# genglongling/EE274_ConvexCaldera_LLM_quantization

Hardware: AMD Instinct MI355X
Metric: weight matrices/sec (4096x4096, rank-128, Q=2-bit) + Frob err vs ref (higher is better)
Workload: dtype f32 (fp16 W in; fp32-grade split-fp16 MFMA products, fp64 small solves; int2 codes)

## Files before the change

### ee274_convexcaldera_llm_quantization_amd/csrc/cq_sgram.hip

```cpp
#include "cq_common.h"

namespace cq {

constexpr int SG_SLICE = 64;

__device__ __forceinline__ uint32_t sg_nz_mask(uint32_t word) {
    const uint32_t x = word ^ 0x55555555u;
    return (x | (x >> 1)) & 0x55555555u;
}

__device__ __forceinline__ uint32_t sg_field(uint32_t word, int u) {
    return (word >> (8 * (u >> 2) + 6 - 2 * (u & 3))) & 3u;
}

__device__ __forceinline__ int sg_u_of_bit(int p) { return 4 * (p >> 3) + ((6 - (p & 7)) >> 1); }

__global__ __launch_bounds__(256) void sgram_count_kernel(const uint8_t* __restrict__ packed, int64_t k, int64_t L,
                                                          int32_t* __restrict__ row_nnz, const _Float16* __restrict__ W,
                                                          const float* __restrict__ qscale,
                                                          const float* __restrict__ wcol, double* __restrict__ row_corr,
                                                          int64_t Lh, int32_t* __restrict__ row_nnz1, int64_t wcs) {
    const int lane = threadIdx.x & 63;
    const int64_t j = (int64_t)blockIdx.x * 4 + (threadIdx.x >> 6);
    const int64_t b = blockIdx.y;
    if (wcol) wcol += b * wcs;
    if (j >= k) return;
    const uint32_t* row = reinterpret_cast<const uint32_t*>(packed + b * (k * L / 4) + j * (L / 4));
    const int64_t nw = L / 16;
    uint32_t cnt = 0, cnt1 = 0;
    double corr = 0.0;
    const double s = W ? (double)qscale[b] : 0.0;
    const _Float16* Wr = W ? W + b * k * L + j * L : nullptr;
    const int64_t nw1 = Lh / 16;
    for (int64_t w = lane; w < nw; w += 64) {
        const uint32_t word = row[w];
        uint32_t nz = sg_nz_mask(word);
        cnt += __popc(nz);
        if (w < nw1) cnt1 += __popc(nz);
        if (W) {
            while (nz) {
                const int p = __builtin_ctz(nz);
                nz &= nz - 1u;
                const int64_t l = 16 * w + sg_u_of_bit(p);
                const double c = (double)((int)((word >> p) & 3u) - 1);
                const double t = s * s - 2.0 * s * c * (double)(float)Wr[l];
                corr += wcol ? (double)wcol[l] * t : t;
            }
        }
    }
    cnt = wave_sum(cnt);
    if (lane == 0) row_nnz[b * k + j] = (int32_t)cnt;
    if (row_nnz1) {
// ... 243 lines not shown
            }
        }
        cntr[r] = cnt;
        __builtin_amdgcn_wave_barrier();
    }
    const int g = lane >> 4, u = lane & 15;
    const int q = (int)((p0 + g) & 15);
    for (int h = 0; h < np; ++h) {
        int myc = 0, mys = 0, mycnt = 0;
        uint32_t* myout = nullptr;
        int T = 0;
#pragma unroll
        for (int r = 0; r < SG_FILL_RW; ++r) {
            const int cn = cntr[r] <= 0 ? 0 : (h ? cntr[r] - c1r[r] : c1r[r]);
            if (g == r) {
                mycnt = cn;
                myout = outr[r] ? outr[r] + (h ? w1r[r] * SG_SLICE : 0) : nullptr;
            }
            T = cn > T ? cn : T;
        }
        if (mycnt > 0) {
            myc = rcb[wv][g][h][u];
            mys = rsb[wv][g][h][u];
        }
        int taken = 0;
        for (int t = 0; t < T; ++t) {
            const int d = (q + t) & 15;
            const int remd = __shfl(myc - taken, 16 * g + d, 64);
            int key = ((myc - taken) << 4) | (15 - u);
#pragma unroll
            for (int o = 8; o > 0; o >>= 1) key = max(key, __shfl_xor(key, o, 64));
            const int sel = remd > 0 ? d : 15 - (key & 15);
            const int at = __shfl(mys + taken, 16 * g + sel, 64);
            if (t < mycnt) {
                if (u == 0) myout[(int64_t)t * SG_SLICE] = grp[wv][g][at];
                if (u == sel) ++taken;
            }
        }
    }
#pragma unroll
    for (int r = 0; r < SG_FILL_RW; ++r) {
        if (!outr[r]) continue;
        const int tot = cntr[r] < 0 ? -cntr[r] : cntr[r];
        for (int64_t t = c1r[r] + lane; t < w1r[r]; t += 64) outr[r][t * SG_SLICE] = 1u;
        if (split) {
            const uint32_t pad = (uint32_t)(Lh << 2) | 1u;
            for (int64_t t = w1r[r] + (tot - c1r[r]) + lane; t < widr[r]; t += 64) outr[r][t * SG_SLICE] = pad;
        }
    }
}

constexpr int SG_PF = 6;
constexpr int SG_WAVES = 16, SG_THREADS = 64 * SG_WAVES;

template <int R>
__device__ __forceinline__ int64_t sg_slab_at(int64_t L, int64_t l, int r) {
    constexpr int PL = R < 4 ? R : 4;
    return (int64_t)(r / PL) * PL * L + l * PL + (r % PL);
}

template <int R>
__device__ __forceinline__ void sg_slice(const float* __restrict__ slab, int64_t L, const uint32_t* __restrict__ ep,
                                         int64_t width, float (&acc)[R], int64_t lbase = 0) {
#pragma unroll
    for (int r = 0; r < R; ++r) acc[r] = 0.f;
    constexpr int PL = R < 4 ? R : 4;
    auto fma_entry = [&](uint32_t e) {
        const float c = (float)((int)(e & 3u) - 1);
        const int64_t l = (int64_t)(e >> 2) - lbase;
#pragma unroll
        for (int pl = 0; pl < R / PL; ++pl) {
            const float* v = slab + (int64_t)pl * PL * L + l * PL;
#pragma unroll
            for (int r = 0; r < PL; ++r) acc[pl * PL + r] = __builtin_fmaf(c, v[r], acc[pl * PL + r]);
        }
    };
    int64_t t = 0;
    if (width >= SG_PF) {
        uint32_t cur[SG_PF];
#pragma unroll
        for (int q = 0; q < SG_PF; ++q) cur[q] = ep[q * SG_SLICE];
        for (t = SG_PF; t + SG_PF <= width; t += SG_PF) {
            uint32_t nxt[SG_PF];
#pragma unroll
            for (int q = 0; q < SG_PF; ++q) nxt[q] = ep[(t + q) * SG_SLICE];
#pragma unroll
            for (int q = 0; q < SG_PF; ++q) fma_entry(cur[q]);
#pragma unroll
            for (int q = 0; q < SG_PF; ++q) cur[q] = nxt[q];
        }
#pragma unroll
        for (int q = 0; q < SG_PF; ++q) fma_entry(cur[q]);
    }
    for (; t < width; ++t) fma_entry(ep[t * SG_SLICE]);
}

template <int R, int NSW, bool SPLIT = false>
__global__ __launch_bounds__(1024) void sgram_spmm_kernel(const _Float16* __restrict__ W, const uint8_t* __restrict__ packed,
                                                         const float* __restrict__ qscale, const float* __restrict__ wcol,
                                                         int64_t k, int64_t L, const uint32_t* __restrict__ ell,
                                                         const int32_t* __restrict__ perm,
                                                         const int64_t* __restrict__ slice_off,
                                                         const int32_t* __restrict__ slice_w1, int64_t Lh,
                                                         int64_t stride_ell, float* __restrict__ P, int64_t wcs) {
    extern __shared__ __attribute__((aligned(16))) float slab[];
    const int64_t b = blockIdx.y;
    if (wcol) wcol += b * wcs;
    const int64_t i0 = (int64_t)blockIdx.x * R;
    const float hs = 0.5f * qscale[b];
    const int64_t KL = k * L;
    const int64_t Ls = SPLIT ? Lh : L;
    constexpr int PL = R < 4 ? R : 4;
    auto stage = [&](int64_t la, int64_t lb) {
#pragma unroll
    for (int pl = 0; pl < R / PL; ++pl) {
        for (int64_t l0 = la + (int64_t)threadIdx.x * 8; l0 < lb; l0 += SG_THREADS * 8) {
            float e[PL][8];
#pragma unroll
            for (int r = 0; r < PL; ++r) {
                const int64_t i = i0 + pl * PL + r;
                if (i < k) {
                    const int64_t el = b * KL + i * L + l0;
                    const uint4 raw = *reinterpret_cast<const uint4*>(W + el);
                    const _Float16* hv = reinterpret_cast<const _Float16*>(&raw);
                    const uint16_t two = *reinterpret_cast<const uint16_t*>(packed + el / 4);
#pragma unroll
                    for (int u = 0; u < 8; ++u) {
                        const uint32_t byte = (u < 4) ? (two & 0xffu) : (two >> 8);
                        const float c = (float)((int)((byte >> (6 - 2 * (u & 3))) & 3u) - 1);
                        e[r][u] = (float)hv[u] - hs * c;
                        if (wcol) e[r][u] *= wcol[l0 + u];
                    }
                } else {
#pragma unroll
                    for (int u = 0; u < 8; ++u) e[r][u] = 0.f;
                }
            }
            const int rot = threadIdx.x & 7;
#pragma unroll
            for (int sh = 1; sh < 8; sh <<= 1) {
                if (rot & sh) {
#pragma unroll
                    for (int r = 0; r < PL; ++r) {
                        float t8[8];
#pragma unroll
                        for (int u = 0; u < 8; ++u) t8[u] = e[r][(u + sh) & 7];
#pragma unroll
                        for (int u = 0; u < 8; ++u) e[r][u] = t8[u];
                    }
                }
            }
#pragma unroll
            for (int u = 0; u < 8; ++u) {
                float* dst = slab + (int64_t)pl * PL * Ls + (l0 - la + ((u + rot) & 7)) * PL;
                if constexpr (PL == 4) *reinterpret_cast<float4*>(dst) = make_float4(e[0][u], e[1][u], e[2][u], e[3][u]);
                else *reinterpret_cast<float2*>(dst) = make_float2(e[0][u], e[1][u]);
            }
        }
    }
    };
    stage(0, SPLIT ? Lh : L);
    __syncthreads();
    const int lane = threadIdx.x & 63, wv = threadIdx.x >> 6;
    const int64_t ns = (k + SG_SLICE - 1) / SG_SLICE;
    const int64_t* so = slice_off + b * (ns + 1);
    const uint32_t* eb = ell + b * stride_ell + lane;
    const int32_t* pm = perm + b * k;
    float* Pb = P + b * k * k;
    if constexpr (NSW > 0) {
        float acc[NSW][R];
#pragma unroll
        for (int q = 0; q < NSW; ++q) {
            const int64_t s = wv + SG_WAVES * q;
            if (s < ns) sg_slice<R>(slab, L, eb + so[s] * SG_SLICE, so[s + 1] - so[s], acc[q]);
        }
        __syncthreads();
#pragma unroll
        for (int q = 0; q < NSW; ++q) {
            const int64_t p = (wv + SG_WAVES * q) * SG_SLICE + lane;
            if (p < k) {
                float* dst = slab + pm[p] * R;
#pragma unroll
                for (int pl = 0; pl < R / PL; ++pl) {
                    if constexpr (PL == 4)
                        *reinterpret_cast<float4*>(dst + 4 * pl) = make_float4(acc[q][4 * pl], acc[q][4 * pl + 1],
                                                                              acc[q][4 * pl + 2], acc[q][4 * pl + 3]);
                    else *reinterpret_cast<float2*>(dst) = make_float2(acc[q][0], acc[q][1]);
                }
            }
        }
        __syncthreads();
        for (int64_t j = threadIdx.x; j < k; j += SG_THREADS) {
            float v[R];
#pragma unroll
            for (int pl = 0; pl < R / PL; ++pl) {
                if constexpr (PL == 4) {
                    const float4 x = *reinterpret_cast<const float4*>(slab + j * R + 4 * pl);
                    v[4 * pl] = x.x; v[4 * pl + 1] = x.y; v[4 * pl + 2] = x.z; v[4 * pl + 3] = x.w;
                } else {
                    const float2 x = *reinterpret_cast<const float2*>(slab + j * R);
                    v[0] = x.x; v[1] = x.y;
                }
            }
#pragma unroll
            for (int r = 0; r < R; ++r)
                if (i0 + r < k) Pb[(i0 + r) * k + j] = v[r];
        }
    } else if constexpr (NSW < 0) {
        float* outb = slab + (int64_t)R * Ls;
        const int32_t* w1 = SPLIT ? slice_w1 + b * ns : nullptr;
        for (int64_t s = wv; s < ns; s += SG_WAVES) {
            float acc[R];
            sg_slice<R>(slab, Ls, eb + so[s] * SG_SLICE, SPLIT ? w1[s] : so[s + 1] - so[s], acc);
            const int64_t p = s * SG_SLICE + lane;
            if (p < k) {
#pragma unroll
                for (int r = 0; r < R; ++r) outb[(int64_t)pm[p] * R + r] = acc[r];
            }
        }
        if constexpr (SPLIT) {
            __syncthreads();
            stage(Lh, L);
            __syncthreads();
            for (int64_t s = wv; s < ns; s += SG_WAVES) {
                float acc[R];
                sg_slice<R>(slab, Ls, eb + (so[s] + w1[s]) * SG_SLICE, so[s + 1] - so[s] - w1[s], acc, Lh);
                const int64_t p = s * SG_SLICE + lane;
                if (p < k) {
#pragma unroll
                    for (int r = 0; r < R; ++r) outb[(int64_t)pm[p] * R + r] += acc[r];
                }
            }
        }
        __syncthreads();
        for (int64_t j = threadIdx.x; j < k; j += SG_THREADS) {
#pragma unroll
            for (int r = 0; r < R; ++r)
                if (i0 + r < k) Pb[(i0 + r) * k + j] = outb[j * R + r];
        }
    } else {
        for (int64_t s = wv; s < ns; s += SG_WAVES) {
            float acc[R];
            sg_slice<R>(slab, L, eb + so[s] * SG_SLICE, so[s + 1] - so[s], acc);
            const int64_t p = s * SG_SLICE + lane;
            if (p < k) {
                const int64_t j = pm[p];
#pragma unroll
                for (int r = 0; r < R; ++r)
                    if (i0 + r < k) Pb[(i0 + r) * k + j] = acc[r];
            }
        }
    }
}

__device__ __forceinline__ float sg_split_scale(double bound) {
    int e = 0;
    if (bound > 0.0 && isfinite(bound)) frexp(bound, &e);
    return ldexpf(1.f, 14 - e);
}

__global__ __launch_bounds__(256) void sgram_combine_kernel(const float* __restrict__ A, const float* __restrict__ P,
                                                            const float* __restrict__ qscale, int64_t k,
                                                            const double* __restrict__ bound, float out_scale,
                                                            _Float16* __restrict__ Gh, _Float16* __restrict__ Gl,
                                                            float* __restrict__ scale_out, float* __restrict__ inv_out,
                                                            float* __restrict__ G32) {
    __shared__ float pt[64][65];
    const int64_t b = blockIdx.y;
    const int64_t nt = k / 64;
    int64_t t = blockIdx.x, I = 0;
    while (t >= nt - I) { t -= nt - I; ++I; }
    const int64_t J = I + t;
    const int64_t I0 = I * 64, J0 = J * 64;
    const float s = qscale[b];
    const float gs = sg_split_scale(bound[b]);
    if (blockIdx.x == 0 && threadIdx.x == 0) {
        scale_out[b] = gs;
        inv_out[b] = 1.f / (gs * out_scale);
    }
    const int64_t KK = k * k;
    const float* Pb = P + b * KK;
    const int tx = threadIdx.x & 15, ty = threadIdx.x >> 4;
    for (int a = ty; a < 64; a += 16) {
        const float4 v = *reinterpret_cast<const float4*>(Pb + (J0 + a) * k + I0 + 4 * tx);
        pt[a][4 * tx] = v.x; pt[a][4 * tx + 1] = v.y; pt[a][4 * tx + 2] = v.z; pt[a][4 * tx + 3] = v.w;
    }
    __syncthreads();
    float g[4][4];
#pragma unroll
    for (int q = 0; q < 4; ++q) {
        const int a = ty + 16 * q;
        const float4 av = *reinterpret_cast<const float4*>(A + b * KK + (I0 + a) * k + J0 + 4 * tx);
        const float4 pv = *reinterpret_cast<const float4*>(Pb + (I0 + a) * k + J0 + 4 * tx);
        const float aa[4] = {av.x, av.y, av.z, av.w}, pp[4] = {pv.x, pv.y, pv.z, pv.w};
#pragma unroll
        for (int u = 0; u < 4; ++u) g[q][u] = aa[u] - s * (pp[u] + pt[4 * tx + u][a]);
// ... 348 lines not shown
    CQ_REQUIRE(bits == 2, "cq_sgram_count: 2-bit codes only");
    CQ_REQUIRE(batch > 0 && batch < 65536 && k > 0 && L > 0 && L % 64 == 0, "cq_sgram_count: bad shape");
    CQ_REQUIRE(!W || (qscale && corr_ws && corr_out), "cq_sgram_count: the norm correction needs qscale, corr_ws, corr_out");
    CQ_REQUIRE(Lh >= L || (Lh > 0 && Lh % 64 == 0 && 2 * Lh >= L && row_nnz1 && slice_w1),
               "cq_sgram_count: an l-split needs Lh % 64 == 0, Lh >= L / 2, row_nnz1 and slice_w1");
    const bool split = Lh < L;
    hipStream_t s = as_stream(stream);
    sgram_count_kernel<<<dim3((unsigned)ceil_div(k, 4), (unsigned)batch), 256, 0, s>>>(
        packed, k, L, row_nnz, reinterpret_cast<const _Float16*>(W), qscale, wcol, corr_ws, split ? Lh : L,
        split ? row_nnz1 : nullptr, wcol_stride);
    sgram_slices_kernel<<<(unsigned)batch, 256, 0, s>>>(row_nnz, k, perm, slice_off, total, W ? corr_ws : nullptr,
                                                        corr_out, split ? row_nnz1 : nullptr, slice_w1);
    return check_launch("cq_sgram_count");
}

int cq_sgram_fill(const uint8_t* packed, int bits, int64_t batch, int64_t k, int64_t L, const int32_t* row_nnz,
                  const int32_t* perm, const int64_t* slice_off, const int32_t* slice_w1, int64_t Lh,
                  int64_t stride_ell, uint32_t* ell, void* stream) {
    CQ_REQUIRE(packed && row_nnz && perm && slice_off && ell, "cq_sgram_fill: null argument");
    CQ_REQUIRE(bits == 2, "cq_sgram_fill: 2-bit codes only");
    CQ_REQUIRE(batch > 0 && batch < 65536 && k > 0 && L > 0 && L % 64 == 0 && L < (1ll << 29),
               "cq_sgram_fill: bad shape");
    CQ_REQUIRE(Lh >= L || (Lh > 0 && Lh % 64 == 0 && 2 * Lh >= L && slice_w1), "cq_sgram_fill: bad l-split");
    sgram_fill_kernel<<<dim3((unsigned)ceil_div(k, 4 * SG_FILL_RW), (unsigned)batch), 256, 0, as_stream(stream)>>>(
        packed, k, L, row_nnz, perm, slice_off, slice_w1, Lh < L ? Lh : L, stride_ell, ell);
    return check_launch("cq_sgram_fill");
}

int cq_sgram_rows(int64_t L) {
    for (int r : {8, 4, 2})
        if ((size_t)L * r * sizeof(float) <= 150 * 1024) return r;
    return 0;
}

int64_t cq_sgram_split(int64_t k, int64_t L) {
    if (cq_sgram_rows(L) != 2 || L % 64) return L;
    const int64_t Lh = ceil_div(L / 2, (int64_t)64) * 64;
    return ((size_t)Lh * 4 + (size_t)k * 4) * sizeof(float) <= 150 * 1024 ? Lh : L;
}

int cq_sgram_spmm(int dtype, const void* W, const uint8_t* packed, const float* qscale, const float* wcol,
                  int64_t wcol_stride, int64_t batch, int64_t k, int64_t L, const uint32_t* ell, const int32_t* perm,
                  const int64_t* slice_off, const int32_t* slice_w1, int64_t Lh, int64_t stride_ell, float* P,
                  void* stream) {
    CQ_REQUIRE(W && packed && qscale && ell && perm && slice_off && P, "cq_sgram_spmm: null argument");
    CQ_REQUIRE(dtype == CQ_F16, "cq_sgram_spmm: fp16 W only");
    CQ_REQUIRE(batch > 0 && batch < 65536 && k > 0 && L % 64 == 0, "cq_sgram_spmm: bad shape");
    hipStream_t s = as_stream(stream);
    const _Float16* Wh = reinterpret_cast<const _Float16*>(W);
    if (Lh < L) {
        CQ_REQUIRE(Lh == cq_sgram_split(k, L) && slice_w1, "cq_sgram_spmm: Lh must be cq_sgram_split(k, L)");
        const size_t lds = ((size_t)Lh * 4 + (size_t)k * 4) * sizeof(float);
        sgram_spmm_kernel<4, -1, true><<<dim3((unsigned)ceil_div(k, 4), (unsigned)batch), SG_THREADS, lds, s>>>(
            Wh, packed, qscale, wcol, k, L, ell, perm, slice_off, slice_w1, Lh, stride_ell, P, wcol_stride);
        return check_launch("cq_sgram_spmm");
    }
    const int R = cq_sgram_rows(L);
    CQ_REQUIRE(R > 0, "cq_sgram_spmm: rows of %lld values do not fit the LDS", (long long)L);
    size_t lds = (size_t)L * R * sizeof(float);
    const dim3 grid((unsigned)ceil_div(k, R), (unsigned)batch);
    const int64_t nsw = ceil_div(ceil_div(k, SG_SLICE), SG_WAVES);
    const bool held = k <= L && nsw * R <= 32 && R == 8;
    const bool ldsout = !held && R < 8 && lds + (size_t)k * R * sizeof(float) <= 150 * 1024;
    if (ldsout) lds += (size_t)k * R * sizeof(float);
#define CQ_SP(RR, NN) sgram_spmm_kernel<RR, NN><<<grid, SG_THREADS, lds, s>>>(Wh, packed, qscale, wcol, k, L, ell, \
                                                                             perm, slice_off, nullptr, L, stride_ell, P, \
                                                                             wcol_stride)
    if (R == 8) {
        if (held) CQ_SP(8, 4); else CQ_SP(8, 0);
    } else if (R == 4) {
        if (ldsout) CQ_SP(4, -1); else CQ_SP(4, 0);
    } else {
        if (ldsout) CQ_SP(2, -1); else CQ_SP(2, 0);
    }
#undef CQ_SP
    return check_launch("cq_sgram_spmm");
}

int cq_sgram_combine(const float* A, const float* P, const float* qscale, int64_t batch, int64_t k,
                     const double* bound, float out_scale, uint16_t* Gh, uint16_t* Gl, float* scale_out,
                     float* inv_out, float* G32, void* stream) {
    CQ_REQUIRE(A && P && qscale && bound && Gh && Gl && scale_out && inv_out, "cq_sgram_combine: null argument");
    CQ_REQUIRE(batch > 0 && batch < 65536 && k > 0 && k % 64 == 0 && out_scale > 0.f, "cq_sgram_combine: bad shape");
    const int64_t nt = k / 64;
    sgram_combine_kernel<<<dim3((unsigned)(nt * (nt + 1) / 2), (unsigned)batch), 256, 0, as_stream(stream)>>>(
        A, P, qscale, k, bound, out_scale, reinterpret_cast<_Float16*>(Gh), reinterpret_cast<_Float16*>(Gl),
        scale_out, inv_out, G32);
    return check_launch("cq_sgram_combine");
}

}
```

### ee274_convexcaldera_llm_quantization_amd/csrc/cq_small.hip

```cpp
#include "cq_common.h"

namespace cq {

constexpr int GT = 64;
constexpr int GK = 32;
constexpr int kGramThreads = 256;

__global__ __launch_bounds__(kGramThreads) void gram_f64_kernel(
    int64_t M, int64_t N, int64_t K, int64_t kchunk, int splits, const float* __restrict__ A,
    int ta, int64_t lda, int64_t sa, const float* __restrict__ B, int tb, int64_t ldb, int64_t sb,
    double* __restrict__ part) {
    __shared__ float As[GK][GT + 1];
    __shared__ float Bs[GK][GT + 1];
    const int64_t b = blockIdx.z / splits;
    const int split = blockIdx.z % splits;
    const int64_t i0 = (int64_t)blockIdx.y * GT, j0 = (int64_t)blockIdx.x * GT;
    const float* Ab = A + b * sa;
    const float* Bb = B + b * sb;
    const int tx = threadIdx.x & 15, ty = threadIdx.x >> 4;
    double acc[4][4];
#pragma unroll
    for (int u = 0; u < 4; ++u)
#pragma unroll
        for (int v = 0; v < 4; ++v) acc[u][v] = 0.0;
// ... 7 lines not shown
            if (gk < kend && gi < M) v = ta ? Ab[gi * lda + gk] : Ab[gk * lda + gi];
            As[kk][ii] = v;
            int jj;
            if (!tb) { kk = e / GT; jj = e % GT; } else { jj = e / GK; kk = e % GK; }
            const int64_t gk2 = k0 + kk, gj = j0 + jj;
            float w = 0.f;
            if (gk2 < kend && gj < N) w = tb ? Bb[gj * ldb + gk2] : Bb[gk2 * ldb + gj];
            Bs[kk][jj] = w;
        }
        __syncthreads();
#pragma unroll 4
        for (int kk = 0; kk < GK; ++kk) {
            double av[4], bv[4];
#pragma unroll
            for (int u = 0; u < 4; ++u) av[u] = (double)As[kk][ty * 4 + u];
#pragma unroll
            for (int v = 0; v < 4; ++v) bv[v] = (double)Bs[kk][tx * 4 + v];
#pragma unroll
            for (int u = 0; u < 4; ++u)
#pragma unroll
                for (int v = 0; v < 4; ++v) acc[u][v] = fma(av[u], bv[v], acc[u][v]);
        }
        __syncthreads();
    }
    double* P = part + ((int64_t)b * splits + split) * M * N;
#pragma unroll
    for (int u = 0; u < 4; ++u)
#pragma unroll
        for (int v = 0; v < 4; ++v) {
            const int64_t i = i0 + ty * 4 + u, j = j0 + tx * 4 + v;
            if (i < M && j < N) P[i * N + j] = acc[u][v];
        }
}

__global__ void gram_reduce_kernel(const double* __restrict__ part, int64_t MN, int splits,
                                   int64_t batch, double* __restrict__ C) {
    const int64_t total = batch * MN;
    for (int64_t e = (int64_t)blockIdx.x * blockDim.x + threadIdx.x; e < total;
         e += (int64_t)gridDim.x * blockDim.x) {
        const int64_t b = e / MN, o = e % MN;
        double s = 0.0;
        for (int t = 0; t < splits; ++t) s += part[(b * splits + t) * MN + o];
        C[e] = s;
    }
}


using f64x4v = __attribute__((ext_vector_type(4))) double;

template <bool TK>
__global__ __launch_bounds__(kGramThreads) void gram_f64_mfma_kernel(
    int64_t M, int64_t N, int64_t K, int64_t kchunk, int splits, const float* __restrict__ A,
    int64_t lda, int64_t sa, const float* __restrict__ B, int64_t ldb, int64_t sb, int sym,
    double* __restrict__ part) {
    constexpr int GP = TK ? GT + 4 : GT + 16;
    __shared__ float As[2][GK][GP];
    __shared__ float Bs[2][GK][GP];
    const int64_t b = blockIdx.z / splits;
    const int split = blockIdx.z % splits;
    if (sym && blockIdx.x < blockIdx.y) return;
    const int64_t i0 = (int64_t)blockIdx.y * GT, j0 = (int64_t)blockIdx.x * GT;
    const float* Ab = A + b * sa;
    const float* Bb = B + b * sb;
    const int t = threadIdx.x, lane = t & 63, wid = t >> 6;
    const int wi = wid >> 1, wj = wid & 1;
    const int lr = t >> 4, lc = (t & 15) * 4;
    const int tr = t >> 3, tk = (t & 7) * 4;
    const int64_t kbeg = split * kchunk, kend = min(K, kbeg + kchunk);
    auto ld4 = [&](const float* base, int64_t ld, int64_t lim, int64_t k, int64_t c0) -> float4 {
        float4 v = make_float4(0.f, 0.f, 0.f, 0.f);
        if (k < kend) {
            const float* src = base + k * ld + c0;
            if (c0 + 3 < lim) v = *reinterpret_cast<const float4*>(src);
            else {
                if (c0 < lim) v.x = src[0];
                if (c0 + 1 < lim) v.y = src[1];
                if (c0 + 2 < lim) v.z = src[2];
            }
        }
        return v;
    };
    f64x4v acc[2][2];
#pragma unroll
    for (int u = 0; u < 2; ++u)
#pragma unroll
        for (int v = 0; v < 2; ++v) acc[u][v] = f64x4v{0.0, 0.0, 0.0, 0.0};
    float4 ra[2], rb[2];
    auto ld4t = [&](const float* base, int64_t ld, int64_t lim, int64_t row, int64_t k) -> float4 {
        float4 v = make_float4(0.f, 0.f, 0.f, 0.f);
        if (row < lim && k < kend) {
            const float* src = base + row * ld + k;
            if (k + 3 < kend) v = *reinterpret_cast<const float4*>(src);
            else {
                v.x = src[0];
                if (k + 1 < kend) v.y = src[1];
                if (k + 2 < kend) v.z = src[2];
            }
        }
        return v;
    };
    auto fetch = [&](int64_t k0) {
#pragma unroll
        for (int h = 0; h < 2; ++h) {
            if constexpr (TK) {
                ra[h] = ld4t(Ab, lda, M, i0 + tr + 32 * h, k0 + tk);
                rb[h] = ld4t(Bb, ldb, N, j0 + tr + 32 * h, k0 + tk);
            } else {
                ra[h] = ld4(Ab, lda, M, k0 + lr + 16 * h, i0 + lc);
                rb[h] = ld4(Bb, ldb, N, k0 + lr + 16 * h, j0 + lc);
            }
        }
    };
    auto stash = [&](int buf) {
#pragma unroll
        for (int h = 0; h < 2; ++h) {
            if constexpr (TK) {
                const int c = tr + 32 * h;
                As[buf][tk + 0][c] = ra[h].x; As[buf][tk + 1][c] = ra[h].y;
                As[buf][tk + 2][c] = ra[h].z; As[buf][tk + 3][c] = ra[h].w;
                Bs[buf][tk + 0][c] = rb[h].x; Bs[buf][tk + 1][c] = rb[h].y;
                Bs[buf][tk + 2][c] = rb[h].z; Bs[buf][tk + 3][c] = rb[h].w;
            } else {
                *reinterpret_cast<float4*>(&As[buf][lr + 16 * h][lc]) = ra[h];
                *reinterpret_cast<float4*>(&Bs[buf][lr + 16 * h][lc]) = rb[h];
            }
        }
    };
    const int nsl = (int)ceil_div(kend - kbeg, GK);
    if (nsl > 0) { fetch(kbeg); stash(0); }
    __syncthreads();
    const int li = lane & 15, lk = lane >> 4;
    for (int sl = 0; sl < nsl; ++sl) {
        const int cur = sl & 1;
        if (sl + 1 < nsl) fetch(kbeg + (int64_t)(sl + 1) * GK);
#pragma unroll
        for (int kk = 0; kk < GK; kk += 4) {
            double a0 = (double)As[cur][kk + lk][32 * wi + li];
            double a1 = (double)As[cur][kk + lk][32 * wi + 16 + li];
            double b0 = (double)Bs[cur][kk + lk][32 * wj + li];
            double b1 = (double)Bs[cur][kk + lk][32 * wj + 16 + li];
            acc[0][0] = __builtin_amdgcn_mfma_f64_16x16x4f64(a0, b0, acc[0][0], 0, 0, 0);
            acc[0][1] = __builtin_amdgcn_mfma_f64_16x16x4f64(a0, b1, acc[0][1], 0, 0, 0);
            acc[1][0] = __builtin_amdgcn_mfma_f64_16x16x4f64(a1, b0, acc[1][0], 0, 0, 0);
            acc[1][1] = __builtin_amdgcn_mfma_f64_16x16x4f64(a1, b1, acc[1][1], 0, 0, 0);
        }
        if (sl + 1 < nsl) stash(1 - cur);
        __syncthreads();
    }
    double* P = part + ((int64_t)b * splits + split) * M * N;
#pragma unroll
    for (int u = 0; u < 2; ++u)
#pragma unroll
        for (int v = 0; v < 2; ++v)
#pragma unroll
            for (int r = 0; r < 4; ++r) {
                const int64_t i = i0 + 32 * wi + 16 * u + lk + 4 * r;
                const int64_t j = j0 + 32 * wj + 16 * v + li;
                if (i < M && j < N) P[i * N + j] = acc[u][v][r];
            }
}

__global__ void gram_reduce_sym_kernel(const double* __restrict__ part, int64_t M, int splits,
                                       int64_t batch, double* __restrict__ C) {
    const int64_t MN = M * M, total = batch * MN;
    for (int64_t e = (int64_t)blockIdx.x * blockDim.x + threadIdx.x; e < total;
         e += (int64_t)gridDim.x * blockDim.x) {
        const int64_t b = e / MN, o = e % MN, i = o / M, j = o % M;
        const int64_t src = (i / GT > j / GT) ? j * M + i : o;
        double s = 0.0;
        for (int t2 = 0; t2 < splits; ++t2) s += part[(b * splits + t2) * MN + src];
        C[e] = s;
    }
}

static int gram_splits(int64_t M, int64_t N, int64_t K, int64_t batch) {
    const int64_t tiles = ceil_div(M, GT) * ceil_div(N, GT) * batch;
    int64_t s = ceil_div(1024, tiles);
    s = std::min<int64_t>(s, std::max<int64_t>(1, K / 256));
    return (int)std::max<int64_t>(1, std::min<int64_t>(s, 64));
}

template <int PPT, int RPT, int JBR, int NTH>
__global__ __launch_bounds__(NTH) void jacobi_reg_kernel(const double* __restrict__ A_all,
                                                                    int p, int max_sweeps, double tol,
                                                                    double* __restrict__ evals,
                                                                    float* __restrict__ V32,
                                                                    double* __restrict__ V64,
                                                                    int* __restrict__ sweeps_out) {
    extern __shared__ __attribute__((aligned(16))) char smem_raw[];
    const int P = p + (p & 1);
    const int H = P / 2;
    double2* csn = reinterpret_cast<double2*>(smem_raw);
    int4* lohi = reinterpret_cast<int4*>(csn + H);
    int* flp = reinterpret_cast<int*>(lohi + H);
    int* seat = flp + H;
    int* seat2 = seat + P;
    int* rnk = seat2 + P;
    double* a = reinterpret_cast<double*>(rnk + P + ((9 * H + 3 * P) & 1));
    __shared__ double red[16];
    __shared__ int stop;
    const int64_t b = blockIdx.x;
    const double* Ag = A_all + b * (int64_t)p * p;
    const int tid = threadIdx.x, lane = tid & 63, wid = tid >> 6;
    const bool wantv = V32 != nullptr || V64 != nullptr;
    const int pg = lane & 31;
    const int rg = 2 * wid + (lane >> 5);
    const int k0 = pg * PPT, x0 = rg * RPT;
    auto pk = [p](int i, int j) -> int {
        if (i > j) { const int t = i; i = j; j = t; }
        return i * p - ((i * (i - 1)) >> 1) + (j - i);
    };
// ... 629 lines not shown
}

__global__ void ritz_prod_final_kernel(const double* part, int nchunks, int64_t p, int64_t r,
                                       const double* theta, const double* ysq, float* out) {
    __shared__ double red[16];
    const int64_t b = blockIdx.x;
    const double t0 = fabs(theta[b * p]), tp = theta[b * p + p - 1];
    double acc = 0.0;
    for (int64_t c = threadIdx.x; c < r; c += blockDim.x) {
        double s = 0.0;
        for (int t = 0; t < nchunks; ++t) s += part[(b * nchunks + t) * r + c];
        const double th = fmax(theta[b * p + c], 0.0);
        const double gap = fmax(th - tp, 1e-3 * t0);
        acc += s * th / (gap * gap);
    }
    acc = wave_sum(acc);
    if ((threadIdx.x & 63) == 0) red[threadIdx.x >> 6] = acc;
    __syncthreads();
    if (threadIdx.x == 0) {
        double a = 0.0;
        for (int i = 0; i < (int)(blockDim.x >> 6); ++i) a += red[i];
        const double y2 = ysq[b];
        out[b] = (float)(y2 > 0 ? sqrt(a / y2) : sqrt(a));
    }
}

}

using namespace cq;

extern "C" {

size_t cq_gram_f64_workspace(int64_t M, int64_t N, int64_t K, int64_t batch) {
    return (size_t)batch * gram_splits(M, N, K, batch) * M * N * sizeof(double);
}

int cq_gram_f64(int64_t M, int64_t N, int64_t K, int64_t batch, const float* A, int trans_a,
                int64_t lda, int64_t stride_a, const float* B, int trans_b, int64_t ldb,
                int64_t stride_b, double* C, void* ws, size_t ws_bytes, void* stream) {
    CQ_REQUIRE(A && B && C && M > 0 && N > 0 && K > 0 && batch > 0, "cq_gram_f64: bad args");
    const int splits = gram_splits(M, N, K, batch);
    if (!ws || ws_bytes < cq_gram_f64_workspace(M, N, K, batch))
        return set_error(CQ_EWORKSPACE, "cq_gram_f64: workspace too small");
    CQ_REQUIRE(batch * splits <= 65535, "cq_gram_f64: batch too large");
    const int64_t kchunk = ceil_div(ceil_div(K, splits), GK) * GK;
    hipStream_t s = as_stream(stream);
    dim3 grid((unsigned)ceil_div(N, GT), (unsigned)ceil_div(M, GT), (unsigned)(batch * splits));
    const int64_t tot = batch * M * N;
    const unsigned rgrid = (unsigned)std::min<int64_t>(ceil_div(tot, 256), 4096);
    const bool al4 = lda % 4 == 0 && ldb % 4 == 0 && stride_a % 4 == 0 && stride_b % 4 == 0 &&
                     reinterpret_cast<uintptr_t>(A) % 16 == 0 && reinterpret_cast<uintptr_t>(B) % 16 == 0;
    if (al4 && trans_a == trans_b) {
        const int sym = (A == B && lda == ldb && stride_a == stride_b && M == N) ? 1 : 0;
        if (trans_a)
            gram_f64_mfma_kernel<true><<<grid, kGramThreads, 0, s>>>(M, N, K, kchunk, splits, A, lda, stride_a, B,
                                                                     ldb, stride_b, sym, reinterpret_cast<double*>(ws));
        else
            gram_f64_mfma_kernel<false><<<grid, kGramThreads, 0, s>>>(M, N, K, kchunk, splits, A, lda, stride_a, B,
                                                                      ldb, stride_b, sym, reinterpret_cast<double*>(ws));
        if (sym)
            gram_reduce_sym_kernel<<<rgrid, 256, 0, s>>>(reinterpret_cast<double*>(ws), M, splits, batch, C);
        else
            gram_reduce_kernel<<<rgrid, 256, 0, s>>>(reinterpret_cast<double*>(ws), M * N, splits, batch, C);
        return check_launch("cq_gram_f64");
    }
    gram_f64_kernel<<<grid, kGramThreads, 0, s>>>(M, N, K, kchunk, splits, A, trans_a, lda,
                                                   stride_a, B, trans_b, ldb, stride_b,
                                                   reinterpret_cast<double*>(ws));
    gram_reduce_kernel<<<rgrid, 256, 0, s>>>(reinterpret_cast<double*>(ws), M * N, splits, batch, C);
    return check_launch("cq_gram_f64");
}

int cq_spd_whiten(double* S, int64_t p, int64_t batch, float* Wt32, double* Wt64, int* info,
                  void* stream) {
    return cq_spd_whiten_rcond(S, p, batch, 1e-30, Wt32, Wt64, info, stream);
}

int cq_spd_whiten_rcond(double* S, int64_t p, int64_t batch, double rcond2, float* Wt32, double* Wt64, int* info,
                        void* stream) {
    CQ_REQUIRE(S && p > 0 && batch > 0 && info && Wt64, "cq_spd_whiten: bad args (Wt64 is required scratch)");
    CQ_REQUIRE(rcond2 >= 0.0, "cq_spd_whiten: rcond2 must be >= 0");
    hipStream_t s = as_stream(stream);
    const size_t wsm = (size_t)(p + 2 * 32 * 33 + 32) * sizeof(double);
    const size_t wlm = wsm + (size_t)32 * wm_pitch((int)p) * sizeof(double);
    CQ_REQUIRE(wsm <= 64 * 1024, "cq_spd_whiten: p too large");
    if (wlm <= 150 * 1024)
        spd_whiten_mfma_kernel<true><<<(unsigned)batch, kWmThreads, wlm, s>>>(S, (int)p, rcond2, Wt64, Wt32, info);
    else
        spd_whiten_mfma_kernel<false><<<(unsigned)batch, kWmThreads, wsm, s>>>(S, (int)p, rcond2, Wt64, Wt32, info);
    return check_launch("cq_spd_whiten");
}

size_t cq_jacobi_workspace(int64_t p, int64_t batch) {
    if (p > kBlockJacobiMinP) return cq::bj_workspace(p, batch);
    return 16;
}

int cq_jacobi_eigh(double* A, int64_t p, int64_t batch, int max_sweeps, double tol, double* evals,
                   float* V32, double* V64, int* sweeps_out, void* ws, size_t ws_bytes,
                   void* stream) {
    CQ_REQUIRE(A && evals && p > 0 && batch > 0 && max_sweeps > 0, "cq_jacobi_eigh: bad args");
    CQ_REQUIRE(p <= 4096, "cq_jacobi_eigh: p too large");
    if (!ws || ws_bytes < cq_jacobi_workspace(p, batch))
        return set_error(CQ_EWORKSPACE, "cq_jacobi_eigh: workspace too small");
    hipStream_t s = as_stream(stream);
    if (p > kBlockJacobiMinP)
        return cq::bj_eigh(A, p, batch, max_sweeps, tol, evals, V32, V64, sweeps_out, ws, ws_bytes, s);
    const size_t lreg = jacobi_reg_bytes((int)p);
    CQ_REQUIRE(lreg <= 160 * 1024, "cq_jacobi_eigh: LDS budget");
    if (p <= 64)
        jacobi_reg_kernel<1, 2, 2, 1024><<<(unsigned)batch, 1024, lreg, s>>>(A, (int)p, max_sweeps, tol, evals, V32, V64, sweeps_out);
    else if (p <= 128)
// ... 75 lines not shown
```

Measured before the change: 350.3.

## Persist sgram SpMM blocks over multiple row tiles with prefetched staging; skip gram reduce

The held-accumulator SpMM path now has each block process up to nb consecutive row tiles. The global loads for the next tile are issued before the sparse FMA phase so they overlap with compute, and the slice metadata is loaded once per block. Staging now uses register lane rotation through alignbit instead of float shuffles. Wave-to-slice assignment is serpentine to balance load. Separately, the fp64 gram kernel writes straight into C, mirroring symmetric tiles, when there is only one split, which removes the reduce launch. The cost is higher register pressure, extra barriers, and a grid that can go below one block per tile.

```diff
diff --git a/ee274_convexcaldera_llm_quantization_amd/csrc/cq_sgram.hip b/ee274_convexcaldera_llm_quantization_amd/csrc/cq_sgram.hip
--- a/ee274_convexcaldera_llm_quantization_amd/csrc/cq_sgram.hip
+++ b/ee274_convexcaldera_llm_quantization_amd/csrc/cq_sgram.hip
@@ -1,3 +1,5 @@
+#include <algorithm>
+
 #include "cq_common.h"
 
 namespace cq {
@@ -347,6 +349,7 @@
 
 constexpr int SG_PF = 6;
 constexpr int SG_WAVES = 16, SG_THREADS = 64 * SG_WAVES;
+constexpr int64_t SG_NB_MAX = 8;
 
 template <int R>
 __device__ __forceinline__ int64_t sg_slab_at(int64_t L, int64_t l, int r) {
@@ -388,6 +391,15 @@
         for (int q = 0; q < SG_PF; ++q) fma_entry(cur[q]);
     }
     for (; t < width; ++t) fma_entry(ep[t * SG_SLICE]);
+}
+
+struct SgStageRegs {
+    uint4 raw[4];
+    uint32_t two[4];
+};
+
+__device__ __forceinline__ int64_t sg_wave_slice(int wv, int q) {
+    return (int64_t)SG_WAVES * q + ((q & 1) ? SG_WAVES - 1 - wv : wv);
 }
 
 template <int R, int NSW, bool SPLIT = false>
@@ -397,146 +409,215 @@
                                                          const int32_t* __restrict__ perm,
                                                          const int64_t* __restrict__ slice_off,
                                                          const int32_t* __restrict__ slice_w1, int64_t Lh,
-                                                         int64_t stride_ell, float* __restrict__ P, int64_t wcs) {
+                                                         int64_t stride_ell, float* __restrict__ P, int64_t wcs, int nb) {
     extern __shared__ __attribute__((aligned(16))) float slab[];
     const int64_t b = blockIdx.y;
+    int tid = threadIdx.x;
     if (wcol) wcol += b * wcs;
-    const int64_t i0 = (int64_t)blockIdx.x * R;
     const float hs = 0.5f * qscale[b];
     const int64_t KL = k * L;
     const int64_t Ls = SPLIT ? Lh : L;
     constexpr int PL = R < 4 ? R : 4;
-    auto stage = [&](int64_t la, int64_t lb) {
-#pragma unroll
-    for (int pl = 0; pl < R / PL; ++pl) {
-        for (int64_t l0 = la + (int64_t)threadIdx.x * 8; l0 < lb; l0 += SG_THREADS * 8) {
-            float e[PL][8];
+    constexpr int NPL = R / PL;
+    auto issue = [&](int64_t i0, int pl, int64_t l0, SgStageRegs& g) {
+#pragma unroll
+        for (int r = 0; r < PL; ++r) {
+            const int64_t i = i0 + pl * PL + r;
+            if (i < k) {
+                const int64_t el = b * KL + i * L + l0;
+                g.raw[r] = *reinterpret_cast<const uint4*>(W + el);
+                g.two[r] = *reinterpret_cast<const uint16_t*>(packed + el / 4);
+            } else {
+                g.raw[r] = make_uint4(0u, 0u, 0u, 0u);
+                g.two[r] = 0x5555u;
+            }
+        }
+    };
+    auto commit = [&](int64_t i0, int pl, int64_t l0, int64_t la, const SgStageRegs& g) {
+        const int rot = tid & 7;
+        uint32_t d[PL][4];
+#pragma unroll
+        for (int r = 0; r < PL; ++r) {
+            const uint32_t x[4] = {g.raw[r].x, g.raw[r].y, g.raw[r].z, g.raw[r].w};
+            uint32_t y[4], z[4];
+#pragma unroll
+            for (int v = 0; v < 4; ++v) y[v] = (rot & 2) ? x[(v + 1) & 3] : x[v];
+#pragma unroll
+            for (int v = 0; v < 4; ++v) z[v] = (rot & 4) ? y[(v + 2) & 3] : y[v];
+#pragma unroll
+            for (int v = 0; v < 4; ++v) d[r][v] = __builtin_amdgcn_alignbit(z[(v + 1) & 3], z[v], 16 * (rot & 1));
+        }
+        float wv[4];
+#pragma unroll
+        for (int u = 0; u < 8; ++u) {
+            const int m = (u + rot) & 7;
+            const int sh = 2 * (m & 4) + 6 - 2 * (m & 3);
+            if (wcol && (u & 3) == 0) {
+#pragma unroll
+                for (int v = 0; v < 4; ++v) wv[v] = wcol[l0 + ((u + v + rot) & 7)];
+            }
+            float e[PL];
 #pragma unroll
             for (int r = 0; r < PL; ++r) {
-                const int64_t i = i0 + pl * PL + r;
-                if (i < k) {
-                    const int64_t el = b * KL + i * L + l0;
-                    const uint4 raw = *reinterpret_cast<const uint4*>(W + el);
-                    const _Float16* hv = reinterpret_cast<const _Float16*>(&raw);
-                    const uint16_t two = *reinterpret_cast<const uint16_t*>(packed + el / 4);
-#pragma unroll
-                    for (int u = 0; u < 8; ++u) {
-                        const uint32_t byte = (u < 4) ? (two & 0xffu) : (two >> 8);
-                        const float c = (float)((int)((byte >> (6 - 2 * (u & 3))) & 3u) - 1);
-                        e[r][u] = (float)hv[u] - hs * c;
-                        if (wcol) e[r][u] *= wcol[l0 + u];
-                    }
-                } else {
-#pragma unroll
-                    for (int u = 0; u < 8; ++u) e[r][u] = 0.f;
-                }
-            }
-            const int rot = threadIdx.x & 7;
-#pragma unroll
-            for (int sh = 1; sh < 8; sh <<= 1) {
-                if (rot & sh) {
-#pragma unroll
-                    for (int r = 0; r < PL; ++r) {
-                        float t8[8];
-#pragma unroll
-                        for (int u = 0; u < 8; ++u) t8[u] = e[r][(u + sh) & 7];
-#pragma unroll
-                        for (int u = 0; u < 8; ++u) e[r][u] = t8[u];
-                    }
-                }
-            }
-#pragma unroll
-            for (int u = 0; u < 8; ++u) {
-                float* dst = slab + (int64_t)pl * PL * Ls + (l0 - la + ((u + rot) & 7)) * PL;
-                if constexpr (PL == 4) *reinterpret_cast<float4*>(dst) = make_float4(e[0][u], e[1][u], e[2][u], e[3][u]);
-                else *reinterpret_cast<float2*>(dst) = make_float2(e[0][u], e[1][u]);
-            }
-        }
-    }
+                const uint16_t hb = (uint16_t)(u & 1 ? d[r][u >> 1] >> 16 : d[r][u >> 1] & 0xffffu);
+                _Float16 h;
+                __builtin_memcpy(&h, &hb, 2);
+                const float c = (float)((int)((g.two[r] >> sh) & 3u) - 1);
+                e[r] = (float)h - hs * c;
+            }
+            if (wcol) {
+#pragma unroll
+                for (int r = 0; r < PL; ++r) e[r] *= wv[u & 3];
+            }
+#pragma unroll
+            for (int r = 0; r < PL; ++r)
+                if (!(i0 + pl * PL + r < k)) e[r] = 0.f;
+            float* dst = slab + (pl * PL * (int)Ls + ((int)(l0 - la) + m) * PL);
+            if constexpr (PL == 4) *reinterpret_cast<float4*>(dst) = make_float4(e[0], e[1], e[2], e[3]);
+            else *reinterpret_cast<float2*>(dst) = make_float2(e[0], e[1]);
+        }
     };
-    stage(0, SPLIT ? Lh : L);
-    __syncthreads();
-    const int lane = threadIdx.x & 63, wv = threadIdx.x >> 6;
+    auto stage = [&](int64_t i0, int64_t la, int64_t lb, int first) {
+        const int nl8 = (int)((lb - la) / 8);
+        for (int it = first + tid; it < NPL * nl8; it += SG_THREADS) {
+            const int pl = NPL > 1 && it >= nl8 ? 1 : 0;
+            const int64_t l0 = la + (int64_t)(it - pl * nl8) * 8;
+            SgStageRegs g;
+            issue(i0, pl, l0, g);
+            commit(i0, pl, l0, la, g);
+        }
+    };
+    const int wv = __builtin_amdgcn_readfirstlane(threadIdx.x >> 6);
+    int lane = threadIdx.x & 63;
     const int64_t ns = (k + SG_SLICE - 1) / SG_SLICE;
     const int64_t* so = slice_off + b * (ns + 1);
-    const uint32_t* eb = ell + b * stride_ell + lane;
+    const uint32_t* eb = ell + b * stride_ell;
     const int32_t* pm = perm + b * k;
     float* Pb = P + b * k * k;
     if constexpr (NSW > 0) {
-        float acc[NSW][R];
+        const int64_t nblk = (k + R - 1) / R;
+        const int64_t blk0 = (int64_t)blockIdx.x * nb;
+        const int nbk = (int)min<int64_t>(nb, nblk - blk0);
+        const int nl8 = (int)(L / 8);
+        int64_t eoff[NSW];
+        int32_t wid[NSW];
+        uint32_t pmv[(NSW + 1) / 2] = {};
 #pragma unroll
         for (int q = 0; q < NSW; ++q) {
-            const int64_t s = wv + SG_WAVES * q;
-            if (s < ns) sg_slice<R>(slab, L, eb + so[s] * SG_SLICE, so[s + 1] - so[s], acc[q]);
-        }
+            const int64_t s = sg_wave_slice(wv, q);
+            eoff[q] = s < ns ? so[s] * SG_SLICE : 0;
+            wid[q] = s < ns ? (int32_t)(so[s + 1] - so[s]) : -1;
+            const int64_t p = s * SG_SLICE + lane;
+            pmv[q / 2] |= (p < k ? (uint32_t)pm[p] : 0xffffu) << (16 * (q & 1));
+        }
+        SgStageRegs g;
+        if (tid < NPL * nl8) issue(blk0 * R, NPL > 1 && tid >= nl8 ? 1 : 0, (int64_t)(tid >= nl8 ? tid - nl8 : tid) * 8, g);
+        for (int n = 0; n < nbk; ++n) {
+            asm volatile("" : "+v"(tid), "+v"(lane));
+#pragma unroll
+            for (int q = 0; q < (NSW + 1) / 2; ++q) asm volatile("" : "+v"(pmv[q]));
+            const bool has0 = tid < NPL * nl8;
+            const int pl0 = NPL > 1 && tid >= nl8 ? 1 : 0;
+            const int64_t l00 = (int64_t)(tid - pl0 * nl8) * 8;
+            const int64_t i0 = (blk0 + n) * R;
+            if (n > 0) __syncthreads();
+            for (int it = tid; it < NPL * nl8; it += SG_THREADS) {
+                asm volatile("" : "+v"(tid));
+                const int pl = NPL > 1 && it >= nl8 ? 1 : 0;
+                const int64_t l0 = (int64_t)(it - pl * nl8) * 8;
+                if (it >= SG_THREADS) issue(i0, pl, l0, g);
+                commit(i0, pl, l0, 0, g);
+            }
+            __syncthreads();
+            if (n + 1 < nbk && has0) issue(i0 + R, pl0, l00, g);
+            float acc[NSW][R];
+#pragma unroll
+            for (int q = 0; q < NSW; ++q)
+                if (wid[q] >= 0) sg_slice<R>(slab, L, eb + eoff[q] + lane, wid[q], acc[q]);
+            __syncthreads();
+#pragma unroll
+            for (int r = 0; r < PL; ++r)
+                asm volatile("" : "+v"(g.raw[r].x), "+v"(g.raw[r].y), "+v"(g.raw[r].z), "+v"(g.raw[r].w), "+v"(g.two[r]));
+#pragma unroll
+            for (int q = 0; q < NSW; ++q) {
+                const uint32_t j = (pmv[q / 2] >> (16 * (q & 1))) & 0xffffu;
+                if (j != 0xffffu) {
+                    float* dst = slab + j * R;
+#pragma unroll
+                    for (int pl = 0; pl < NPL; ++pl) {
+                        if constexpr (PL == 4)
+                            *reinterpret_cast<float4*>(dst + 4 * pl) = make_float4(acc[q][4 * pl], acc[q][4 * pl + 1],
+                                                                                  acc[q][4 * pl + 2], acc[q][4 * pl + 3]);
+                        else *reinterpret_cast<float2*>(dst) = make_float2(acc[q][0], acc[q][1]);
+                    }
+                }
+            }
+            __syncthreads();
+            for (int64_t j = tid; j < k; j += SG_THREADS) {
+                float v[R];
+#pragma unroll
+                for (int pl = 0; pl < NPL; ++pl) {
+                    if constexpr (PL == 4) {
+                        const float4 x = *reinterpret_cast<const float4*>(slab + j * R + 4 * pl);
+                        v[4 * pl] = x.x; v[4 * pl + 1] = x.y; v[4 * pl + 2] = x.z; v[4 * pl + 3] = x.w;
+                    } else {
+                        const float2 x = *reinterpret_cast<const float2*>(slab + j * R);
+                        v[0] = x.x; v[1] = x.y;
+                    }
+                }
+#pragma unroll
+                for (int r = 0; r < R; ++r)
+                    if (i0 + r < k) Pb[(i0 + r) * k + j] = v[r];
+            }
+        }
+    } else if constexpr (NSW < 0) {
+        const int64_t i0 = (int64_t)blockIdx.x * R;
+        stage(i0, 0, Ls, 0);
         __syncthreads();
-#pragma unroll
-        for (int q = 0; q < NSW; ++q) {
-            const int64_t p = (wv + SG_WAVES * q) * SG_SLICE + lane;
+        float* outb = slab + (int64_t)R * Ls;
+        const int32_t* w1 = SPLIT ? slice_w1 + b * ns : nullptr;
+        for (int q = 0; SG_WAVES * q < ns; ++q) {
+            const int64_t s = sg_wave_slice(wv, q);
+            if (s >= ns) continue;
+            float acc[R];
+            sg_slice<R>(slab, Ls, eb + so[s] * SG_SLICE + lane, SPLIT ? w1[s] : so[s + 1] - so[s], acc);
+            const int64_t p = s * SG_SLICE + lane;
             if (p < k) {
-                float* dst = slab + pm[p] * R;
-#pragma unroll
-                for (int pl = 0; pl < R / PL; ++pl) {
-                    if constexpr (PL == 4)
-                        *reinterpret_cast<float4*>(dst + 4 * pl) = make_float4(acc[q][4 * pl], acc[q][4 * pl + 1],
-                                                                              acc[q][4 * pl + 2], acc[q][4 * pl + 3]);
-                    else *reinterpret_cast<float2*>(dst) = make_float2(acc[q][0], acc[q][1]);
+#pragma unroll
+                for (int r = 0; r < R; ++r) outb[(int64_t)pm[p] * R + r] = acc[r];
+            }
+        }
+        if constexpr (SPLIT) {
+            __syncthreads();
+            stage(i0, Lh, L, 0);
+            __syncthreads();
+            for (int q = 0; SG_WAVES * q < ns; ++q) {
+                const int64_t s = sg_wave_slice(wv, q);
+                if (s >= ns) continue;
+                float acc[R];
+                sg_slice<R>(slab, Ls, eb + (so[s] + w1[s]) * SG_SLICE + lane, so[s + 1] - so[s] - w1[s], acc, Lh);
+                const int64_t p = s * SG_SLICE + lane;
+                if (p < k) {
+#pragma unroll
+                    for (int r = 0; r < R; ++r) outb[(int64_t)pm[p] * R + r] += acc[r];
                 }
             }
         }
         __syncthreads();
         for (int64_t j = threadIdx.x; j < k; j += SG_THREADS) {
-            float v[R];
-#pragma unroll
-            for (int pl = 0; pl < R / PL; ++pl) {
-                if constexpr (PL == 4) {
-                    const float4 x = *reinterpret_cast<const float4*>(slab + j * R + 4 * pl);
-                    v[4 * pl] = x.x; v[4 * pl + 1] = x.y; v[4 * pl + 2] = x.z; v[4 * pl + 3] = x.w;
-                } else {
-                    const float2 x = *reinterpret_cast<const float2*>(slab + j * R);
-                    v[0] = x.x; v[1] = x.y;
-                }
-            }
-#pragma unroll
-            for (int r = 0; r < R; ++r)
-                if (i0 + r < k) Pb[(i0 + r) * k + j] = v[r];
-        }
-    } else if constexpr (NSW < 0) {
-        float* outb = slab + (int64_t)R * Ls;
-        const int32_t* w1 = SPLIT ? slice_w1 + b * ns : nullptr;
-        for (int64_t s = wv; s < ns; s += SG_WAVES) {
-            float acc[R];
-            sg_slice<R>(slab, Ls, eb + so[s] * SG_SLICE, SPLIT ? w1[s] : so[s + 1] - so[s], acc);
-            const int64_t p = s * SG_SLICE + lane;
-            if (p < k) {
-#pragma unroll
-                for (int r = 0; r < R; ++r) outb[(int64_t)pm[p] * R + r] = acc[r];
-            }
-        }
-        if constexpr (SPLIT) {
-            __syncthreads();
-            stage(Lh, L);
-            __syncthreads();
-            for (int64_t s = wv; s < ns; s += SG_WAVES) {
-                float acc[R];
-                sg_slice<R>(slab, Ls, eb + (so[s] + w1[s]) * SG_SLICE, so[s + 1] - so[s] - w1[s], acc, Lh);
-                const int64_t p = s * SG_SLICE + lane;
-                if (p < k) {
-#pragma unroll
-                    for (int r = 0; r < R; ++r) outb[(int64_t)pm[p] * R + r] += acc[r];
-                }
-            }
-        }
-        __syncthreads();
-        for (int64_t j = threadIdx.x; j < k; j += SG_THREADS) {
 #pragma unroll
             for (int r = 0; r < R; ++r)
                 if (i0 + r < k) Pb[(i0 + r) * k + j] = outb[j * R + r];
         }
     } else {
-        for (int64_t s = wv; s < ns; s += SG_WAVES) {
+        const int64_t i0 = (int64_t)blockIdx.x * R;
+        stage(i0, 0, L, 0);
+        __syncthreads();
+        for (int q = 0; SG_WAVES * q < ns; ++q) {
+            const int64_t s = sg_wave_slice(wv, q);
+            if (s >= ns) continue;
             float acc[R];
-            sg_slice<R>(slab, L, eb + so[s] * SG_SLICE, so[s + 1] - so[s], acc);
+            sg_slice<R>(slab, L, eb + so[s] * SG_SLICE + lane, so[s + 1] - so[s], acc);
             const int64_t p = s * SG_SLICE + lane;
             if (p < k) {
                 const int64_t j = pm[p];
@@ -991,20 +1072,23 @@
         CQ_REQUIRE(Lh == cq_sgram_split(k, L) && slice_w1, "cq_sgram_spmm: Lh must be cq_sgram_split(k, L)");
         const size_t lds = ((size_t)Lh * 4 + (size_t)k * 4) * sizeof(float);
         sgram_spmm_kernel<4, -1, true><<<dim3((unsigned)ceil_div(k, 4), (unsigned)batch), SG_THREADS, lds, s>>>(
-            Wh, packed, qscale, wcol, k, L, ell, perm, slice_off, slice_w1, Lh, stride_ell, P, wcol_stride);
+            Wh, packed, qscale, wcol, k, L, ell, perm, slice_off, slice_w1, Lh, stride_ell, P, wcol_stride, 1);
         return check_launch("cq_sgram_spmm");
     }
     const int R = cq_sgram_rows(L);
     CQ_REQUIRE(R > 0, "cq_sgram_spmm: rows of %lld values do not fit the LDS", (long long)L);
     size_t lds = (size_t)L * R * sizeof(float);
-    const dim3 grid((unsigned)ceil_div(k, R), (unsigned)batch);
+    dim3 grid((unsigned)ceil_div(k, R), (unsigned)batch);
     const int64_t nsw = ceil_div(ceil_div(k, SG_SLICE), SG_WAVES);
     const bool held = k <= L && nsw * R <= 32 && R == 8;
     const bool ldsout = !held && R < 8 && lds + (size_t)k * R * sizeof(float) <= 150 * 1024;
     if (ldsout) lds += (size_t)k * R * sizeof(float);
+    const int64_t nblk = ceil_div(k, R);
+    const int nb = held ? (int)std::max<int64_t>(1, std::min<int64_t>({SG_NB_MAX, nblk * batch / (2 * kCUs), nblk})) : 1;
+    grid.x = (unsigned)ceil_div(nblk, nb);
 #define CQ_SP(RR, NN) sgram_spmm_kernel<RR, NN><<<grid, SG_THREADS, lds, s>>>(Wh, packed, qscale, wcol, k, L, ell, \
                                                                              perm, slice_off, nullptr, L, stride_ell, P, \
-                                                                             wcol_stride)
+                                                                             wcol_stride, nb)
     if (R == 8) {
         if (held) CQ_SP(8, 4); else CQ_SP(8, 0);
     } else if (R == 4) {
diff --git a/ee274_convexcaldera_llm_quantization_amd/csrc/cq_small.hip b/ee274_convexcaldera_llm_quantization_amd/csrc/cq_small.hip
--- a/ee274_convexcaldera_llm_quantization_amd/csrc/cq_small.hip
+++ b/ee274_convexcaldera_llm_quantization_amd/csrc/cq_small.hip
@@ -83,7 +83,7 @@
 __global__ __launch_bounds__(kGramThreads) void gram_f64_mfma_kernel(
     int64_t M, int64_t N, int64_t K, int64_t kchunk, int splits, const float* __restrict__ A,
     int64_t lda, int64_t sa, const float* __restrict__ B, int64_t ldb, int64_t sb, int sym,
-    double* __restrict__ part) {
+    double* __restrict__ part, double* __restrict__ C) {
     constexpr int GP = TK ? GT + 4 : GT + 16;
     __shared__ float As[2][GK][GP];
     __shared__ float Bs[2][GK][GP];
@@ -178,7 +178,8 @@
         if (sl + 1 < nsl) stash(1 - cur);
         __syncthreads();
     }
-    double* P = part + ((int64_t)b * splits + split) * M * N;
+    double* P = C ? C + (int64_t)b * M * N : part + ((int64_t)b * splits + split) * M * N;
+    const bool mirror = C && sym && blockIdx.x != blockIdx.y;
 #pragma unroll
     for (int u = 0; u < 2; ++u)
 #pragma unroll
@@ -187,7 +188,11 @@
             for (int r = 0; r < 4; ++r) {
                 const int64_t i = i0 + 32 * wi + 16 * u + lk + 4 * r;
                 const int64_t j = j0 + 32 * wj + 16 * v + li;
-                if (i < M && j < N) P[i * N + j] = acc[u][v][r];
+                if (i < M && j < N) {
+                    const double x = C ? 0.0 + acc[u][v][r] : acc[u][v][r];
+                    P[i * N + j] = x;
+                    if (mirror) P[j * N + i] = x;
+                }
             }
 }
 
@@ -923,12 +928,16 @@
                      reinterpret_cast<uintptr_t>(A) % 16 == 0 && reinterpret_cast<uintptr_t>(B) % 16 == 0;
     if (al4 && trans_a == trans_b) {
         const int sym = (A == B && lda == ldb && stride_a == stride_b && M == N) ? 1 : 0;
+        double* direct = splits == 1 ? C : nullptr;
         if (trans_a)
             gram_f64_mfma_kernel<true><<<grid, kGramThreads, 0, s>>>(M, N, K, kchunk, splits, A, lda, stride_a, B,
-                                                                     ldb, stride_b, sym, reinterpret_cast<double*>(ws));
+                                                                     ldb, stride_b, sym, reinterpret_cast<double*>(ws),
+                                                                     direct);
         else
             gram_f64_mfma_kernel<false><<<grid, kGramThreads, 0, s>>>(M, N, K, kchunk, splits, A, lda, stride_a, B,
-                                                                      ldb, stride_b, sym, reinterpret_cast<double*>(ws));
+                                                                      ldb, stride_b, sym, reinterpret_cast<double*>(ws),
+                                                                      direct);
+        if (direct) return check_launch("cq_gram_f64");
         if (sym)
             gram_reduce_sym_kernel<<<rgrid, 256, 0, s>>>(reinterpret_cast<double*>(ws), M, splits, batch, C);
         else
```

Measured after the change: 357.5 (median of 6 runs). +2.1%, better.
